# parklab/emsar

Hardware: AMD Instinct MI355X
Metric: EM iterations/s (higher is better)
Workload: dtype f64

## Files before the change

### emsar_amd/csrc/emsar_hip.hip

```cpp
#include <hip/hip_runtime.h>

#include <algorithm>
#include <chrono>
#include <cmath>
#include <cstdio>
#include <cstdlib>
#include <cstring>
#include <new>
#include <numeric>
#include <string>
#include <vector>

#include "../../include/emsar_hip.h"
#include "layout.hpp"
#include "layout_tiled.hpp"
#include "sets.hpp"
#include "boot_rng.hpp"
#include "internal.hpp"
#include "devmem.hpp"
#include "fit_index.hpp"

#include "kernels_common.hpp"
#include "kernels_csr.hpp"
#include "kernels_tiled.hpp"
#include "kernels_vector.hpp"
#include "kernels_sets.hpp"
#include "kernels_presence.hpp"
#include "kernels_cluster.hpp"
#include "kernels_boot.hpp"
#include "kernels_genes.hpp"
#include "kernels_quant.hpp"
#include "kernels_isoforms.hpp"
#include "kernels_fit.hpp"

using emsar::DevBuf;
using emsar::PinBuf;


// ... 17 lines not shown
};

struct GeneMap {
    bool have_genes = false;
    int32_t n_genes = 0;
    int64_t n_gene_chunks = 0, n_gene_multi = 0;
    DevBuf<int32_t> d_gene_blk;
    int32_t *d_gene_tx = nullptr, *d_chunk_beg = nullptr, *d_chunk_out = nullptr, *d_gene_multi = nullptr, *d_gene_of_lib = nullptr;
};

struct AdjEuma {
    DevBuf<int32_t> d_euma_t; int32_t nfl = 0; DevBuf<double> d_wf, d_adj;
};

struct RowWeights { DevBuf<int32_t> d_wgt, d_left_wgt; };

struct LayoutDev {
    DevBuf<void> d_row_ptr;
    DevBuf<int32_t> d_col;
    emsar::TiledLayout TL;
    DevBuf<Tile> d_tiles;
    DevBuf<Tile> d_utiles; int unit_stride = 1;
    DevBuf<uint32_t> d_units; int64_t n_units = 0;
    DevBuf<uint32_t> d_fwd, d_bwd;
    DevBuf<int32_t> d_far;
    DevBuf<uint64_t> d_left_ptr; DevBuf<int32_t> d_left_col; DevBuf<double> d_left_val;
    int64_t n_left = 0, n_tiles = 0, n_slots = 0;
    DevBuf<double> d_u;
    DevBuf<double> d_rowval;
};

struct TxVectors {
    DevBuf<double> d_den, d_acc;
    DevBuf<double> d_th[5];
    DevBuf<double> d_tmp[3];
    DevBuf<int32_t> d_itmp;
};

struct emsar_hip_ctx {
    int device = 0;
    int n_cu = 64;
    hipStream_t stream = nullptr;
    hipEvent_t ev0 = nullptr, ev1 = nullptr, ev2 = nullptr;
    hipStream_t side[3] = {nullptr, nullptr, nullptr};
    hipEvent_t ev_fork = nullptr, ev_join[3] = {nullptr, nullptr, nullptr};
    hipEvent_t ev_c0 = nullptr, ev_c1 = nullptr;
    std::string err;
    bool have_structure = false, have_sample = false;
    int layout = EMSAR_LAYOUT_CSR;
    int64_t n_rows = 0, nnz = 0;
    int32_t n_tx = 0;
    bool ptr64 = false;
    LayoutDev lay;
    TxVectors vec;
    GeneMap genes;
    AdjEuma euma;
    FitDev fit;
    bool weighted = false;
    RowWeights rw;
    SetsDev sets;
    double loglik_const = 0.0;
    DevBuf<Scal> d_scal;
    PinBuf<Scal> h_scal;
    int64_t bytes_formula = 0, bytes_stored = 0;
    int64_t tl_fwd_slots = 0, tl_n_fslices = 0;
    bool use_graph = true;
    bool det = false;
    double fx_mass = 0.0, fx_ll = 0.0;
    DevBuf<double> d_sqpart;
    int update_grid = 1024;
    int sq_grid = 256;
    int weighted_unit = 1;
    int tiled_multi = 1;
    std::vector<uint64_t> h_row_ptr;
    std::vector<int32_t> h_col, h_wgt;
    double sets_build_ms = 0.0;
};

namespace {

#define HIPCHK(call)                                                                                   \
    do {                                                                                               \
        hipError_t e_ = (call);                                                                        \
        if (e_ != hipSuccess) {                                                                        \
            ctx->err = std::string(#call) + ": " + hipGetErrorString(e_);                              \
            return e_ == hipErrorOutOfMemory ? EMSAR_HIP_ERR_OOM : EMSAR_HIP_ERR_HIP;                   \
        }                                                                                              \
    } while (0)

// ... 152 lines not shown
}



int choose_layout(int64_t n_rows, int &layout, bool &merge_rows) {
    merge_rows = (layout & EMSAR_LAYOUT_FLAG_MERGE_ROWS) != 0;
    layout &= ~EMSAR_LAYOUT_FLAG_MERGE_ROWS;
    if (layout != EMSAR_LAYOUT_AUTO && layout != EMSAR_LAYOUT_CSR && layout != EMSAR_LAYOUT_TILED) return EMSAR_HIP_ERR_ARG;
    if (layout == EMSAR_LAYOUT_AUTO) {
        layout = (n_rows < ((int64_t)1 << 32)) ? EMSAR_LAYOUT_TILED : EMSAR_LAYOUT_CSR;
        if (const char *e = getenv("EMSAR_HIP_LAYOUT")) { int v = atoi(e); if ((v == 1 || v == 3) && (v == 1 || n_rows < ((int64_t)1 << 32))) layout = v; }
    }
    return merge_rows && layout != EMSAR_LAYOUT_TILED ? EMSAR_HIP_ERR_ARG : EMSAR_HIP_OK;
}

struct UploadTrace {
    const bool on = getenv("EMSAR_HIP_DEBUG") != nullptr;
    const std::chrono::steady_clock::time_point t0 = std::chrono::steady_clock::now();
    void say(const char *what) const {
        if (on) fprintf(stderr, "upload_structure: %s after %.0f ms\n", what, std::chrono::duration<double, std::milli>(std::chrono::steady_clock::now() - t0).count());
    }
};

int upload_tiled(emsar_hip_ctx *ctx, const uint64_t *row_ptr, const int32_t *col_idx, bool merge_rows, const UploadTrace &trace) {
    auto &L = ctx->lay.TL;
    LayoutDev &D = ctx->lay;
    const size_t T = (size_t)ctx->n_tx;
    const int brc = emsar::build_tiled(ctx->n_rows, ctx->n_tx, row_ptr, col_idx, L, merge_rows);
    if (brc != 0) { ctx->err = "TILED layout builder: code " + std::to_string(brc); return EMSAR_HIP_ERR_ARG; }
    trace.say("layout built");
    D.n_tiles = (int64_t)L.tiles.size(); D.n_slots = L.n_slots(); D.n_left = (int64_t)L.left_row.size();
    HIPCHK(D.d_tiles.upload(L.tiles.data(), L.tiles.size()));
    HIPCHK(D.d_units.upload(L.unit_first.data(), L.unit_first.size()));
    D.n_units = L.unit_first.empty() ? 0 : (int64_t)L.unit_first.size() - 1;
    {
        emsar::UnitTables U;
        emsar::build_unit_tables(L, U);
        D.unit_stride = U.stride;
        HIPCHK(D.d_utiles.upload(U.utiles.data(), U.utiles.size()));
    }
    HIPCHK(D.d_fwd.upload(L.fwd.data(), L.fwd.size()));
    HIPCHK(D.d_bwd.upload(L.bwd.data(), L.bwd.size()));
    HIPCHK(D.d_far.upload(L.far_tid.data(), L.far_tid.size()));
    HIPCHK(D.d_left_ptr.upload(L.left_ptr.data(), L.left_ptr.size()));
    HIPCHK(D.d_left_col.upload(L.left_col.data(), L.left_col.size()));
    HIPCHK(D.d_u.alloc(T));
    HIPCHK(hipMemset(D.d_u, 0, T * 8));
    ctx->bytes_stored = (int64_t)L.fwd.size() * 4 + (int64_t)L.bwd.size() * 4 + (int64_t)L.far_tid.size() * 4 +
                        (int64_t)L.tiles.size() * 64 + (int64_t)L.left_col.size() * 4 + (int64_t)L.left_ptr.size() * 8;
    ctx->tl_fwd_slots = L.padded_slots; ctx->tl_n_fslices = L.n_fslices;
    emsar::u32_vec().swap(L.fwd); emsar::u32_vec().swap(L.bwd);
    std::vector<int32_t>().swap(L.left_col);
    HIPCHK(set_tiled_lds_attributes());
    { const char *pe = getenv("EMSAR_HIP_WEIGHTED_UNIT"); ctx->weighted_unit = pe ? atoi(pe) : 1; }
    { const char *pe = getenv("EMSAR_HIP_TILED_MULTI"); ctx->tiled_multi = pe ? atoi(pe) : 1; }
    { const char *pe = getenv("EMSAR_HIP_UPDATE_GRID"); if (pe && atoi(pe) >= 1) ctx->update_grid = atoi(pe); }
    { const char *pe = getenv("EMSAR_HIP_SQ_GRID"); if (pe && atoi(pe) >= 1) ctx->sq_grid = atoi(pe); }
    return EMSAR_HIP_OK;
}

int upload_csr(emsar_hip_ctx *ctx, const uint64_t *row_ptr, const int32_t *col_idx) {
    const int64_t n_rows = ctx->n_rows;
    if (ctx->ptr64) {
// ... 287 lines not shown
    HIPCHK(hipGetLastError());
    HIPCHK(hipMemcpyAsync(out, ctx->euma.d_adj, (size_t)ctx->n_rows * 8, hipMemcpyDeviceToHost, ctx->stream));
    HIPCHK(hipStreamSynchronize(ctx->stream));
    return EMSAR_HIP_OK;
}

int emsar_hip_get_info(const emsar_hip_ctx *ctx, emsar_hip_info *o) {
    if (!ctx || !o) return EMSAR_HIP_ERR_ARG;
    if (!ctx->have_structure) return EMSAR_HIP_ERR_STATE;
    memset(o, 0, sizeof(*o));
    o->n_rows = ctx->n_rows; o->nnz = ctx->nnz; o->n_tx = ctx->n_tx; o->device_id = ctx->device;
    o->layout = ctx->layout | ((ctx->layout == EMSAR_LAYOUT_TILED && ctx->lay.TL.merged) ? EMSAR_LAYOUT_FLAG_MERGE_ROWS : 0);
    if (ctx->layout == EMSAR_LAYOUT_TILED) {
        o->n_chunks = ctx->lay.n_tiles; o->n_slices = ctx->tl_n_fslices; o->padded_entries = ctx->tl_fwd_slots;
        o->far_entries = ctx->lay.TL.far_entries; o->window = emsar::kTileDict;
        o->tiled_entries = ctx->lay.TL.tiled_entries; o->tiled_ids = ctx->lay.TL.tiled_ids; o->renumbered = ctx->lay.TL.renum.applied ? 1 : 0;
        o->n_units = ctx->lay.n_units;
    }
    o->bytes_per_pass = ctx->bytes_formula;
    o->stored_bytes_per_pass = stored_bytes(ctx);
    return EMSAR_HIP_OK;
}

int emsar_hip_layout_selfcheck_tiled(int64_t n_rows, int32_t n_tx, const uint64_t *row_ptr, const int32_t *col_idx,
                                     int merge_rows, emsar_hip_info *info_out) {
    try {
        if (emsar::validate_csr(n_rows, n_tx, row_ptr, col_idx) != 0) return EMSAR_HIP_ERR_ARG;
        emsar::TiledLayout L;
        if (emsar::build_tiled(n_rows, n_tx, row_ptr, col_idx, L, merge_rows != 0) != 0) return EMSAR_HIP_ERR_ARG;
        int rc = emsar::check_tiled(L, row_ptr, col_idx);
        if (rc == 0) { emsar::UnitTables U; emsar::build_unit_tables(L, U); rc = emsar::check_unit_tables(L, U); }
        if (info_out) {
            memset(info_out, 0, sizeof(*info_out));
            info_out->n_rows = n_rows; info_out->nnz = L.nnz; info_out->n_tx = n_tx;
            info_out->layout = EMSAR_LAYOUT_TILED | (L.merged ? EMSAR_LAYOUT_FLAG_MERGE_ROWS : 0);
            info_out->n_chunks = (int64_t)L.tiles.size();
            info_out->n_slices = L.n_fslices;
            info_out->padded_entries = L.padded_slots; info_out->far_entries = L.far_entries; info_out->window = emsar::kTileDict;
            info_out->stored_bytes_per_pass = (int64_t)L.fwd.size() * 4 + (int64_t)L.bwd.size() * 4 +
                                              (int64_t)L.far_tid.size() * 4 + (int64_t)L.tiles.size() * 64 + (int64_t)L.left_col.size() * 4;
            info_out->bytes_per_pass = (int64_t)L.single_row.size();
            info_out->tiled_entries = L.tiled_entries; info_out->tiled_ids = L.tiled_ids; info_out->renumbered = L.renum.applied ? 1 : 0;
            info_out->n_units = L.unit_first.empty() ? 0 : (int64_t)L.unit_first.size() - 1;
        }
        return rc == 0 ? EMSAR_HIP_OK : EMSAR_HIP_ERR_ARG - 100 + rc;
    } catch (const std::bad_alloc &) { return EMSAR_HIP_ERR_OOM; }
// ... 32 lines not shown
```

### emsar_amd/csrc/kernels_tiled.hpp

```cpp
#pragma once

namespace {

#ifndef EMSAR_UE_BATCH
#define EMSAR_UE_BATCH 6
#endif
#ifndef EMSAR_UM_BATCH
#define EMSAR_UM_BATCH 6
#endif
constexpr int kTiledThreads = 256;
constexpr int kRPL = emsar::kRowsPerLane;
constexpr int kTiledWr = emsar::kTileSliceRows + 8;
constexpr int kTiledDictPad = emsar::kDictEntries;
constexpr int kBlk = emsar::kBlk;
constexpr int kTiledLdsDoubles = 2 * kTiledDictPad + emsar::kTileSlices * kTiledWr;

__device__ __forceinline__ double lds_at(const double *base, unsigned byte_off) {
    return *reinterpret_cast<const double *>(reinterpret_cast<const char *>(base) + byte_off);
}
__device__ __forceinline__ unsigned id_off(unsigned dword, int f) { return ((dword >> (10 * f)) & 0x3FFu) << 3; }

typedef int v4i_t __attribute__((ext_vector_type(4)));
__device__ __forceinline__ void load8_clamped(int4 (&q)[8], const int4 *e, int n) {
#pragma unroll
    for (int j = 0; j < 8; j++) {
        const v4i_t t = __builtin_nontemporal_load(reinterpret_cast<const v4i_t *>(e + (size_t)(j < n ? j : n - 1) * 64));
        q[j] = make_int4(t.x, t.y, t.z, t.w);
    }
}

template <int LO>
__device__ __forceinline__ void load4_clamped(int4 (&q)[8], const int4 *e, int n) {
#pragma unroll
    for (int j = LO; j < LO + 4; j++) {
        const v4i_t t = __builtin_nontemporal_load(reinterpret_cast<const v4i_t *>(e + (size_t)(j < n ? j : n - 1) * 64));
        q[j] = make_int4(t.x, t.y, t.z, t.w);
    }
}

typedef __attribute__((address_space(3))) const double lds_cdouble;
__device__ __forceinline__ unsigned lds_byte_addr(const void *p) { return (unsigned)(uintptr_t)p; }
template <int F>
__device__ __forceinline__ unsigned lds_id_addr(unsigned dword, unsigned base ) {
    unsigned a;
    asm("v_bfe_u32 %0, %1, %2, 10\n\tv_lshl_add_u32 %0, %0, 3, %3" : "=v"(a) : "v"(dword), "i"(10 * F), "s"(base));
    return a;
}
__device__ __forceinline__ double lds_ld(unsigned a) { return *reinterpret_cast<lds_cdouble *>(a); }
template <int H>
__device__ __forceinline__ void lds_addr6(const int4 t, unsigned base, unsigned (&a)[6]) {
    const unsigned d0 = (unsigned)(H ? t.z : t.x), d1 = (unsigned)(H ? t.w : t.y);
    a[0] = lds_id_addr<0>(d0, base); a[1] = lds_id_addr<1>(d0, base); a[2] = lds_id_addr<2>(d0, base);
    a[3] = lds_id_addr<0>(d1, base); a[4] = lds_id_addr<1>(d1, base); a[5] = lds_id_addr<2>(d1, base);
}

template <int BATCH = 12, int LO = 0, int HI = 8>
__device__ __forceinline__ void fwd_sum_regs(const int4 (&q)[8], int n, unsigned th_base, double (&S)[kRPL]) {
#pragma unroll
// ... 519 lines not shown
    BlockDict D;
    int4 A[8], B[8];
    block_dict_far_issue(far_tid + T.far_off, (int)T.far_n, D);
    block_dict_issue<MODE>(T, theta, D);
    if (W.has_slice) {
        load8_clamped(A, W.e, W.k < 8 ? W.k : 8);
        if (W.m > 0) load8_clamped(B, W.b, W.m < 8 ? W.m : 8);
    }
    if (V.lane < 8) V.w_s[emsar::kTileSliceRows + V.lane] = 0.0;
    LlAcc ll;
    tiled_stage<WEIGHTED, MODE, 0, N>(V, (int)blockIdx.x, T, W, A, B, D, ll);
    if (MODE == MODE_EM_LL) {
        double t = block_sum<kTiledThreads>(ll_value(ll), red);
        if (threadIdx.x == 0 && t != 0.0) ll_add(ll_out, t, fx.ll);
    }
}

template <bool WEIGHTED, int MODE, bool STAMP = false>
__global__ __launch_bounds__(kTiledThreads, 4) void k_pass_tiled_unit(const Tile *__restrict__ utiles, int stride, const int32_t *__restrict__ far_tid,
                                                                   const uint32_t *__restrict__ fwd, const uint32_t *__restrict__ bwd,
                                                                   
                                                                   const int32_t *__restrict__ wgt, const double *__restrict__ theta,
                                                                   double *__restrict__ acc, double *__restrict__ ll_out, Fx fx,
                                                                   unsigned long long *stamps = nullptr) {
    extern __shared__ __attribute__((aligned(16))) double lds[];
    __shared__ double red[kTiledThreads / 64];
    const int lane = threadIdx.x & 63;
    const int wave = __builtin_amdgcn_readfirstlane(threadIdx.x >> 6);
    double *th_w = lds, *acc_w = lds + kTiledDictPad, *w_s = lds + 2 * kTiledDictPad + wave * kTiledWr;
    unsigned long long ts0 = 0, ts1 = 0, ts2 = 0, te = 0, tm = 0, tr0 = 0;
    if (STAMP) { ts0 = stamp_now(); tr0 = stamp_real(); }
    const Tile *tiles = utiles + (size_t)blockIdx.x * (size_t)stride;
    BlockDict D;
    DTile T = tile_load(tiles);
    block_dict_far_issue(far_tid + T.far_off, (int)T.far_n, D);
    const int dict_near_n = (int)T.near_n, dict_lo = T.lo, dict_far_n = (int)T.far_n;
    const uint32_t dict_far_off = T.far_off;
    TileWave W = tile_wave(T, unit_slice(T, wave), lane, fwd, bwd);
    int4 A[8], B[8];
    load8_clamped(A, W.has_slice ? W.e : reinterpret_cast<const int4 *>(fwd), W.has_slice ? (W.k < 8 ? W.k : 8) : 1);
    block_dict_issue<MODE>(T, theta, D);
    if (lane < 8) w_s[emsar::kTileSliceRows + lane] = 0.0;
    block_dict_store(T, D, th_w, acc_w);
    vm_loads_landed();
    if (STAMP) ts1 = stamp_now();
    __syncthreads();
    if (STAMP) ts2 = stamp_now();
    LlAcc ll;
    int n_done = 0;
    for (int t = 0;; t++) {
        unsigned long long ta = 0, tb = 0;
        if (STAMP) ta = stamp_now();
        if (W.has_slice) {
            load8_clamped(B, W.b, W.m < 8 ? W.m : 8);
            tile_e_step<WEIGHTED, MODE>(W, A, (size_t)T.row_base + (size_t)W.slice * emsar::kTileSliceRows + lane, wgt, th_w, w_s, lane, ll);
// ... 54 lines not shown
```

### emsar_amd/csrc/layout_tiled.hpp

```cpp
#pragma once
#include <algorithm>
#include <thread>
#include <atomic>
#include <chrono>
#include <cstdio>
#include <cstddef>
#include <cstdint>
#include <cstdlib>
#include <cstring>
#include <functional>
#include <memory>
#include <new>
#include <system_error>
#include <utility>
#include <vector>

#include "layout.hpp"
#include "renumber.hpp"

namespace emsar {

constexpr int kTileSlices = 4;
constexpr int kRowsPerLane = 12;
constexpr int kTileSliceRows = 64 * kRowsPerLane;
// ... 859 lines not shown
struct UnitTables { std::vector<Tile> utiles; int stride = 1; };
inline void build_unit_tables(const TiledLayout &L, UnitTables &U) {
    const size_t nu = L.unit_first.empty() ? 0 : L.unit_first.size() - 1;
    int stride = 1;
    for (size_t u = 0; u < nu; u++) stride = std::max(stride, (int)(L.unit_first[u + 1] - L.unit_first[u]));
    U.stride = stride;
    Tile none;
    std::memset(&none, 0, sizeof none);
    U.utiles.assign(nu * (size_t)stride, none);
    for (size_t u = 0; u < nu; u++) {
        const uint32_t a = L.unit_first[u], b = L.unit_first[u + 1];
        for (uint32_t t = a; t < b; t++) U.utiles[u * (size_t)stride + (t - a)] = L.tiles[t];
    }
    if (getenv("EMSAR_HIP_DEBUG")) {
        std::vector<uint32_t> cnt((size_t)L.n_tx, 0);
        size_t slots = 0, with = 0; uint32_t mx = 0;
        for (size_t u = 0; u < nu; u++) {
            const Tile &T = L.tiles[L.unit_first[u]];
            for (uint32_t f = 0; f < T.far_n; f++) { cnt[(size_t)L.far_tid[(size_t)T.far_off + f]]++; slots++; }
        }
        for (uint32_t c : cnt) { with += c > 0; mx = std::max(mx, c); }
        fprintf(stderr, "unit tables: %zu units, stride %d, %zu far slots of %zu transcripts (most per transcript %u)\n", nu, stride, slots, with, mx);
    }
}

inline int check_unit_tables(const TiledLayout &L, const UnitTables &U) {
    const size_t nu = L.unit_first.empty() ? 0 : L.unit_first.size() - 1;
    if (U.stride < 1 || U.stride > kUnitMaxTiles) return -40;
    if (U.utiles.size() != nu * (size_t)U.stride) return -41;
    for (size_t u = 0; u < nu; u++) {
        const uint32_t a = L.unit_first[u], b = L.unit_first[u + 1];
        if (b - a > (uint32_t)U.stride) return -42;
        for (int j = 0; j < U.stride; j++) {
            const Tile &X = U.utiles[u * (size_t)U.stride + (size_t)j];
            if (a + (uint32_t)j < b) { if (std::memcmp(&X, &L.tiles[a + (uint32_t)j], sizeof(Tile)) != 0) return -43; }
            else if (X.n_slices != 0) return -44;
        }
    }
    return 0;
}

inline int check_tiled(const TiledLayout &L, const uint64_t *row_ptr, const int32_t *col_idx_in) {
    if (const int ext = check_tiled_extents(L)) return ext;
    std::vector<int32_t> mapped;
    const int32_t *col_idx = col_idx_in;
    if (!L.new_of_old.empty()) {
// ... 98 lines not shown
```

### emsar_amd/csrc/pass_launch.hpp

```cpp

namespace {

constexpr int64_t kPairMinTiles = 2048;
enum PassFamily { FAMILY_TILE, FAMILY_MULTI, FAMILY_UNIT };
struct PassKernel { PassFamily family; bool weighted; int mode; int n_multi;  };

PassKernel choose_pass_kernel(bool weighted, int mode, int64_t n_tiles, int tiled_multi, int weighted_unit) {
    if (mode == MODE_SCATTER) return {FAMILY_TILE, false, MODE_SCATTER, 0};
    const bool above = tiled_multi == 1 && n_tiles > kPairMinTiles;
    if (!weighted && (tiled_multi >= 2 || above)) {
        if (tiled_multi == 1 || tiled_multi == 5) return {FAMILY_UNIT, false, mode, 0};
        return {FAMILY_MULTI, false, mode, tiled_multi == 3 ? 3 : tiled_multi == 4 ? 4 : 2};
    }
    if (weighted && (weighted_unit == 2 || (weighted_unit == 1 && mode == MODE_EM)) && (tiled_multi == 5 || above)) {
        return {FAMILY_UNIT, true, mode, 0};
    }
    return {FAMILY_TILE, weighted, mode, 0};
}

template <bool B> using BoolC = std::integral_constant<bool, B>;
template <int M> using ModeC = std::integral_constant<int, M>;
template <class F> void with_em_mode(int mode, const F &f) { if (mode == MODE_EM_LL) f(ModeC<MODE_EM_LL>()); else f(ModeC<MODE_EM>()); }
template <class F> void with_em_variant(bool weighted, int mode, const F &f) {
    if (weighted) with_em_mode(mode, [&](auto md) { f(BoolC<true>(), md); });
    else with_em_mode(mode, [&](auto md) { f(BoolC<false>(), md); });
}

constexpr size_t kTiledLds = (size_t)kTiledLdsDoubles * sizeof(double);
struct PassArgs { const double *theta; double *acc, *ll_out; Fx fx; };

template <bool WT, int MD> void launch_tile(BoolC<WT>, ModeC<MD>, emsar_hip_ctx *ctx, const PassArgs &a) {
    const LayoutDev &L = ctx->lay;
    hipLaunchKernelGGL((k_pass_tiled<WT, MD>), dim3((unsigned)L.n_tiles), dim3(kTiledThreads), kTiledLds, ctx->stream, L.d_tiles, L.d_fwd, L.d_bwd,
                       L.d_far, ctx->rw.d_wgt, L.d_rowval, a.theta, a.acc, a.ll_out, a.fx);
}
template <bool WT, int MD, int N> void launch_multi(BoolC<WT>, ModeC<MD>, std::integral_constant<int, N>, emsar_hip_ctx *ctx, const PassArgs &a) {
    const LayoutDev &L = ctx->lay;
    hipLaunchKernelGGL((k_pass_tiled_multi<WT, MD, N>), dim3((unsigned)((L.n_tiles + N - 1) / N)), dim3(kTiledThreads), kTiledLds, ctx->stream, L.d_tiles,
                       (int)L.n_tiles, L.d_fwd, L.d_bwd, L.d_far, ctx->rw.d_wgt, a.theta, a.acc, a.ll_out, a.fx);
}
template <bool WT, int MD> void launch_unit(BoolC<WT>, ModeC<MD>, emsar_hip_ctx *ctx, const PassArgs &a) {
    const LayoutDev &L = ctx->lay;
    hipLaunchKernelGGL((k_pass_tiled_unit<WT, MD>), dim3((unsigned)L.n_units), dim3(kTiledThreads), kTiledLds, ctx->stream, L.d_utiles, L.unit_stride,
                       L.d_far, L.d_fwd, L.d_bwd, ctx->rw.d_wgt, a.theta, a.acc, a.ll_out, a.fx);
}
template <class PT, bool WT, int MD>
void launch_csr_rows(emsar_hip_ctx *ctx, unsigned max_grid, int64_t n_rows, const PT *row_ptr, const int32_t *col, const int32_t *wgt, const double *val, const PassArgs &a) {
    hipLaunchKernelGGL((k_pass_csr<PT, WT, MD>), dim3((unsigned)std::min<int64_t>((n_rows + 255) / 256, max_grid)), dim3(256), 0, ctx->stream, n_rows, row_ptr,
                       col, wgt, val, a.theta, a.acc, a.ll_out, a.fx);
}
template <bool WT, int MD> void launch_left(BoolC<WT>, ModeC<MD>, emsar_hip_ctx *ctx, const PassArgs &a) {
    const LayoutDev &L = ctx->lay;
    launch_csr_rows<uint64_t, WT, MD>(ctx, 8192, L.n_left, L.d_left_ptr, L.d_left_col, ctx->rw.d_left_wgt, L.d_left_val, a);
}
template <bool WT, int MD> void launch_csr(BoolC<WT>, ModeC<MD>, emsar_hip_ctx *ctx, const PassArgs &a) {
    const LayoutDev &L = ctx->lay;
    if (ctx->ptr64) launch_csr_rows<uint64_t, WT, MD>(ctx, 256 * 32, ctx->n_rows, (const uint64_t *)L.d_row_ptr.get(), L.d_col, ctx->rw.d_wgt, L.d_rowval, a);
    else launch_csr_rows<uint32_t, WT, MD>(ctx, 256 * 32, ctx->n_rows, (const uint32_t *)L.d_row_ptr.get(), L.d_col, ctx->rw.d_wgt, L.d_rowval, a);
}

hipError_t set_tiled_lds_attributes() {
    hipError_t e = hipSuccess;
    auto set = [&](auto *kernel) { if (e == hipSuccess) e = hipFuncSetAttribute((const void *)kernel, hipFuncAttributeMaxDynamicSharedMemorySize, (int)kTiledLds); };
    set(k_pass_tiled<false, MODE_SCATTER>);
    for (const bool weighted : {false, true})
        for (const int mode : {MODE_EM, MODE_EM_LL})
            with_em_variant(weighted, mode, [&](auto wt, auto md) { set(k_pass_tiled<wt(), md()>); set(k_pass_tiled_unit<wt(), md()>); });
// ... 54 lines not shown
        for (size_t w = 0; w < nw; w++) sum += (double)h[w * 8 + (size_t)i];
        out[i] = sum / (double)nw;
    }
    return EMSAR_HIP_OK;
}

}

extern "C" {

int emsar_hip_debug_tiled_stamps(emsar_hip_ctx *ctx, double *out) {
    if (!ctx || !out || ctx->layout != EMSAR_LAYOUT_TILED || !ctx->have_sample || ctx->weighted || ctx->lay.n_tiles == 0) return EMSAR_HIP_ERR_STATE;
    const LayoutDev &L = ctx->lay;
    const size_t nw = (size_t)L.n_tiles * (kTiledThreads / 64);
    std::vector<unsigned long long> h;
    const int rc = stamped_launch(ctx, (const void *)k_pass_tiled<false, MODE_EM, true>, nw, nw * 8, [&](unsigned long long *d) {
        hipLaunchKernelGGL((k_pass_tiled<false, MODE_EM, true>), dim3((unsigned)L.n_tiles), dim3(kTiledThreads), kTiledLds, ctx->stream, L.d_tiles, L.d_fwd, L.d_bwd,
                           L.d_far, ctx->rw.d_wgt, L.d_rowval, ctx->vec.d_th[0], ctx->vec.d_acc, &ctx->d_scal->ll[3].s[0].v, Fx{0.0, 0.0}, d);
    }, h, out);
    if (rc == EMSAR_HIP_OK) out[7] = (double)L.n_tiles;
    return rc;
}

int emsar_hip_debug_unit_stamps(emsar_hip_ctx *ctx, double *out, unsigned long long *timeline ) {
    if (!ctx || !out || ctx->layout != EMSAR_LAYOUT_TILED || !ctx->have_sample || ctx->weighted || ctx->lay.n_units == 0) return EMSAR_HIP_ERR_STATE;
    const LayoutDev &L = ctx->lay;
    const size_t nw = (size_t)L.n_units * (kTiledThreads / 64);
    std::vector<unsigned long long> h;
    const int rc = stamped_launch(ctx, (const void *)k_pass_tiled_unit<false, MODE_EM, true>, nw, nw * 8 + (size_t)L.n_units * 4, [&](unsigned long long *d) {
        hipLaunchKernelGGL((k_pass_tiled_unit<false, MODE_EM, true>), dim3((unsigned)L.n_units), dim3(kTiledThreads), kTiledLds, ctx->stream, L.d_utiles, L.unit_stride,
                           L.d_far, L.d_fwd, L.d_bwd, ctx->rw.d_wgt, ctx->vec.d_th[0], ctx->vec.d_acc, &ctx->d_scal->ll[3].s[0].v, Fx{0.0, 0.0}, d);
    }, h, out);
    if (rc != EMSAR_HIP_OK) return rc;
    if (timeline) std::copy(h.begin() + (std::ptrdiff_t)(nw * 8), h.end(), timeline);
    out[7] = (double)L.n_units;
    return EMSAR_HIP_OK;
}

int emsar_hip_debug_pass_kernel(int weighted, int mode, int64_t n_tiles, int tiled_multi, int weighted_unit, char *out, size_t cap) {
    if (!out || mode < MODE_EM || mode > MODE_SCATTER) return EMSAR_HIP_ERR_ARG;
    const PassKernel k = choose_pass_kernel(weighted != 0, mode, n_tiles, tiled_multi, weighted_unit);
    const char *const wt = k.weighted ? "true" : "false";
    const int len = k.family == FAMILY_MULTI  ? snprintf(out, cap, "k_pass_tiled_multi<%s, %d, %d>", wt, k.mode, k.n_multi)
                    : k.family == FAMILY_UNIT ? snprintf(out, cap, "k_pass_tiled_unit<%s, %d>", wt, k.mode)
                                              : snprintf(out, cap, "k_pass_tiled<%s, %d>", wt, k.mode);
    return len >= 0 && (size_t)len < cap ? EMSAR_HIP_OK : EMSAR_HIP_ERR_ARG;
}

}
```

### emsar_amd/hip.py

```python
import ctypes as C
import os

import numpy as np

_PKG = os.path.dirname(os.path.abspath(__file__))
_LIB_PATH = os.environ.get("EMSAR_HIP_LIB") or os.path.join(_PKG, "libemsar_hip.so")
_lib = None

LAYOUT_AUTO, LAYOUT_CSR, LAYOUT_TILED = 0, 1, 3
FLAG_MERGE_ROWS = 0x100

SYMBOLS = [
    "emsar_hip_create", "emsar_hip_destroy", "emsar_hip_strerror", "emsar_hip_last_error",
    "emsar_hip_upload_structure", "emsar_hip_upload_sample", "emsar_hip_solve",
    "emsar_hip_reset_theta", "emsar_hip_set_theta", "emsar_hip_get_theta", "emsar_hip_run_passes",
    "emsar_hip_ieuma", "emsar_hip_normalise", "emsar_hip_get_info",
    "emsar_hip_layout_selfcheck_tiled", "emsar_hip_sets_selfcheck", "emsar_hip_upload_euma", "emsar_hip_adj_euma", "emsar_hip_collapse_rows",
    "emsar_hip_set_deterministic", "emsar_hip_bootstrap", "emsar_hip_bootstrap_weights", "emsar_hip_bootstrap_draw_host",
    "emsar_hip_set_gene_map", "emsar_hip_gene_sums", "emsar_hip_bootstrap_genes",
    "emsar_hip_subsample", "emsar_hip_subsample_weights", "emsar_hip_subsample_draw_host",
    "emsar_hip_bootstrap_quantiles", "emsar_hip_quantiles_host",
    "emsar_hip_isoform_usage", "emsar_hip_isoform_usage_host", "emsar_hip_bootstrap_isoforms",
    "emsar_hip_model_fit", "emsar_hip_model_fit_host",
    "emsar_hip_presence", "emsar_hip_presence_pvalue_host",
]

PRESENCE_STATUS = ("TESTED", "ABSENT", "ESSENTIAL", "OUTSIDE", "NOT_RESIDENT", "UNCONVERGED")


class EmsarHipError(RuntimeError):
    def __init__(self, status, what, detail=""):
        self.status = status
        super().__init__("%s: %s (status %d)%s" % (what, _strerror(status), status, (" -- " + detail) if detail else ""))


class EmParams(C.Structure):
    _fields_ = [("max_iter", C.c_int32), ("accel", C.c_int32), ("tol", C.c_double), ("abs_floor", C.c_double),
                ("check_every", C.c_int32), ("set_mode", C.c_int32), ("count_floor", C.c_double), ("zero_cut", C.c_double), ("abs_step", C.c_double),
                ("newton_after", C.c_int32), ("reserved0", C.c_int32)]
# ... 96 lines not shown
    if _lib is not None:
        return _lib
    if not os.path.exists(_LIB_PATH):
        raise EmsarHipError(-4, "load_library", "%s missing: run python -m emsar_amd._build" % _LIB_PATH)
    L = C.CDLL(_LIB_PATH)
    vp, u64p, i32p, f64p = C.c_void_p, C.POINTER(C.c_uint64), C.POINTER(C.c_int32), C.POINTER(C.c_double)
    L.emsar_hip_create.argtypes = [C.POINTER(vp), C.c_int]
    L.emsar_hip_destroy.argtypes = [vp]
    L.emsar_hip_destroy.restype = None
    L.emsar_hip_strerror.argtypes = [C.c_int]
    L.emsar_hip_strerror.restype = C.c_char_p
    L.emsar_hip_last_error.argtypes = [vp]
    L.emsar_hip_last_error.restype = C.c_char_p
    L.emsar_hip_upload_structure.argtypes = [vp, C.c_int64, C.c_int32, u64p, i32p, C.c_int]
    L.emsar_hip_upload_sample.argtypes = [vp, i32p, f64p, f64p]
    L.emsar_hip_solve.argtypes = [vp, C.POINTER(EmParams), f64p, C.POINTER(EmStats)]
    L.emsar_hip_reset_theta.argtypes = [vp]
    L.emsar_hip_set_theta.argtypes = [vp, f64p]
    L.emsar_hip_get_theta.argtypes = [vp, f64p]
    L.emsar_hip_run_passes.argtypes = [vp, C.c_int32, C.POINTER(C.c_float), f64p]
    L.emsar_hip_ieuma.argtypes = [vp, f64p, f64p]
    L.emsar_hip_normalise.argtypes = [vp, f64p, f64p, C.c_int64, f64p, f64p, i32p]
    L.emsar_hip_get_info.argtypes = [vp, C.POINTER(Info)]
    L.emsar_hip_layout_selfcheck_tiled.argtypes = [C.c_int64, C.c_int32, u64p, i32p, C.c_int, C.POINTER(Info)]
    L.emsar_hip_set_deterministic.argtypes = [vp, C.c_int]
    L.emsar_hip_set_deterministic.restype = C.c_int
    L.emsar_hip_collapse_rows.argtypes = [vp, C.c_int64, C.c_int32, u64p, i32p, i32p, C.POINTER(C.c_int64), u64p, i32p, i32p, i32p,
                                          C.POINTER(CollapseStats)]
    L.emsar_hip_upload_euma.argtypes = [vp, i32p, C.c_int32]
    L.emsar_hip_adj_euma.argtypes = [vp, f64p, f64p]
    L.emsar_hip_sets_selfcheck.argtypes = [C.c_int64, C.c_int32, u64p, i32p, i32p, C.POINTER(SetsInfo)]
    L.emsar_hip_bootstrap.argtypes = [vp, C.POINTER(EmParams), C.c_uint64, C.c_int32, C.c_int32, f64p, f64p, f64p, f64p, C.POINTER(BootStats)]
    L.emsar_hip_bootstrap_weights.argtypes = [vp, C.c_uint64, C.c_int32, i32p]
    L.emsar_hip_bootstrap_draw_host.argtypes = [C.c_uint64, C.c_int32, C.c_int64, i32p, i32p]
    L.emsar_hip_set_gene_map.argtypes = [vp, C.c_int32, i32p]
    L.emsar_hip_gene_sums.argtypes = [vp, C.c_int32, f64p, f64p]
    L.emsar_hip_bootstrap_genes.argtypes = [vp, C.POINTER(EmParams), C.c_uint64, C.c_int32, C.c_int32, f64p, f64p, f64p, f64p,
                                            f64p, f64p, f64p, C.POINTER(BootStats)]
    L.emsar_hip_subsample.argtypes = [vp, C.POINTER(EmParams), C.c_uint64, C.c_int32, f64p, C.c_int32, f64p, f64p, f64p, f64p, f64p, f64p,
                                      f64p, f64p, f64p, C.POINTER(SubsampleStats)]
    L.emsar_hip_subsample_weights.argtypes = [vp, C.c_uint64, C.c_int32, C.c_double, i32p]
    L.emsar_hip_subsample_draw_host.argtypes = [C.c_uint64, C.c_int32, C.c_double, C.c_int64, i32p, i32p]
    L.emsar_hip_bootstrap_quantiles.argtypes = [vp, C.POINTER(EmParams), C.c_uint64, C.c_int32, C.c_int32, C.c_int32, f64p] + [f64p] * 12 + [
        C.POINTER(BootStats), C.POINTER(QuantileStats)]
    L.emsar_hip_quantiles_host.argtypes = [C.c_int32, C.c_int64, f64p, C.c_int32, f64p, f64p]
    L.emsar_hip_isoform_usage.argtypes = [vp, C.c_int32, f64p, f64p, i32p]
# ... 442 lines not shown
        ms = C.c_float(0)
        ll = C.c_double(0)
        self._chk(self._L.emsar_hip_run_passes(self._h, n, C.byref(ms), C.byref(ll) if want_loglik else None),
                  "run_passes")
        return (ms.value, ll.value) if want_loglik else ms.value

    def ieuma(self, row_L):
        row_L = _arr(row_L, np.float64)
        out = np.zeros(self.n_tx)
        self._chk(self._L.emsar_hip_ieuma(self._h, _p(row_L, C.c_double), _p(out, C.c_double)), "ieuma")
        return out

    def normalise(self, mean_fpkm, ieuma, total_read_count):
        m, ie = _arr(mean_fpkm, np.float64), _arr(ieuma, np.float64)
        tpm, ir = np.zeros(self.n_tx), np.zeros(self.n_tx)
        iri = np.zeros(self.n_tx, dtype=np.int32)
        self._chk(self._L.emsar_hip_normalise(self._h, _p(m, C.c_double), _p(ie, C.c_double), int(total_read_count),
                                              _p(tpm, C.c_double), _p(ir, C.c_double), _p(iri, C.c_int32)), "normalise")
        return tpm, ir, iri

    def info(self):
        i = Info()
        self._chk(self._L.emsar_hip_get_info(self._h, C.byref(i)), "get_info")
        return i.as_dict()
```

### include/emsar_hip.h

```cpp
#ifndef EMSAR_HIP_H
#define EMSAR_HIP_H

#include <stdint.h>

#ifdef __cplusplus
extern "C" {
#endif

typedef struct emsar_hip_ctx emsar_hip_ctx;

typedef enum {
    EMSAR_HIP_OK = 0,
    EMSAR_HIP_ERR_ARG = -1,
    EMSAR_HIP_ERR_NO_DEVICE = -2,
    EMSAR_HIP_ERR_OOM = -3,
    EMSAR_HIP_ERR_HIP = -4,
    EMSAR_HIP_ERR_STATE = -5,
    EMSAR_HIP_ERR_NUMERIC = -6
} emsar_hip_status;

typedef enum {
    EMSAR_LAYOUT_AUTO = 0,
    EMSAR_LAYOUT_CSR = 1,
    EMSAR_LAYOUT_TILED = 3
// ... 185 lines not shown
int emsar_hip_presence(emsar_hip_ctx *ctx, const emsar_em_params *p, int32_t n_query, const int32_t *query_tids ,
                       const emsar_presence_outputs *out , emsar_presence_stats *stats );
int emsar_hip_presence_pvalue_host(int64_t n, const double *lambda, double *p_out);

typedef struct {
    int64_t n_rows, nnz;
    int32_t n_tx;
    int32_t layout;
    int64_t n_chunks;
    int64_t n_slices;
    int64_t padded_entries;
    int64_t far_entries;
    int32_t window;
    int32_t device_id;
    int64_t bytes_per_pass;
    int64_t stored_bytes_per_pass;
    int64_t tiled_entries;
    int64_t tiled_ids;
    int64_t n_units;
    int32_t renumbered;
    int32_t reserved0;
} emsar_hip_info;
int emsar_hip_get_info(const emsar_hip_ctx *ctx, emsar_hip_info *out);

int emsar_hip_layout_selfcheck_tiled(int64_t n_rows, int32_t n_tx, const uint64_t *row_ptr, const int32_t *col_idx,
                                     int merge_rows, emsar_hip_info *info_out);

typedef struct {
    int64_t n_components;
    int64_t sets_resident[3];
    int64_t max_lds_bytes[3];
    int64_t sets_streamed;
    int64_t tids_closed, tids_resident, tids_streamed;
    int64_t rows_in, rows_stored;
    int64_t sets_cluster, tids_cluster, max_lds_cluster;
} emsar_hip_sets_info;
int emsar_hip_sets_selfcheck(int64_t n_rows, int32_t n_tx, const uint64_t *row_ptr, const int32_t *col_idx,
                             const int32_t *row_weight, emsar_hip_sets_info *info_out);

#ifdef __cplusplus
}
#endif
#endif
```

Baseline: 9616.

## Alternate tiled unit sweep order across passes to reuse cached index data

Result: no change. 9687 (median of 6 runs) (+0.7%).

```diff
diff --git a/emsar_amd/csrc/emsar_hip.hip b/emsar_amd/csrc/emsar_hip.hip
--- a/emsar_amd/csrc/emsar_hip.hip
+++ b/emsar_amd/csrc/emsar_hip.hip
@@ -14,6 +14,7 @@
 #include "../../include/emsar_hip.h"
 #include "layout.hpp"
 #include "layout_tiled.hpp"
+#include "sweep_order.hpp"
 #include "sets.hpp"
 #include "boot_rng.hpp"
 #include "internal.hpp"
@@ -77,6 +78,8 @@
     DevBuf<Tile> d_tiles;
     DevBuf<Tile> d_utiles; int unit_stride = 1;
     DevBuf<uint32_t> d_units; int64_t n_units = 0;
+    DevBuf<uint32_t> d_order[2];
+    int64_t sweep_head_units = 0, sweep_group_units = 0, sweep_reuse_bytes = 0;
     DevBuf<uint32_t> d_fwd, d_bwd;
     DevBuf<int32_t> d_far;
     DevBuf<uint64_t> d_left_ptr; DevBuf<int32_t> d_left_col; DevBuf<double> d_left_val;
@@ -120,6 +123,7 @@
     int64_t bytes_formula = 0, bytes_stored = 0;
     int64_t tl_fwd_slots = 0, tl_n_fslices = 0;
     bool use_graph = true;
+    int sweep_phase = 0;
     bool det = false;
     double fx_mass = 0.0, fx_ll = 0.0;
     DevBuf<double> d_sqpart;
@@ -318,6 +322,39 @@
     }
 };
 
+emsar::SweepKnobs read_sweep_knobs() {
+    auto knob = [](const char *name, int64_t dflt) { const char *e = getenv(name); const long long v = e ? atoll(e) : -1; return e && v >= 0 ? (int64_t)v : dflt; };
+    emsar::SweepKnobs K;
+    K.reuse_bytes = 1024 * knob("EMSAR_HIP_SWEEP_REUSE_KB", emsar::kSweepReuseKB);
+    K.head_bytes = 1024 * knob("EMSAR_HIP_SWEEP_HEAD_KB", emsar::kSweepHeadKB);
+    K.min_units = knob("EMSAR_HIP_SWEEP_MIN_UNITS", emsar::kSweepMinUnits);
+    return K;
+}
+int upload_sweep_order(emsar_hip_ctx *ctx, const emsar::SweepKnobs &K, bool same_phase = false) {
+    LayoutDev &D = ctx->lay;
+    ctx->sweep_phase = 0;
+    D.d_order[0] = DevBuf<uint32_t>(); D.d_order[1] = DevBuf<uint32_t>();
+    D.sweep_head_units = D.sweep_group_units = D.sweep_reuse_bytes = 0;
+    std::vector<int64_t> work, bytes;
+    emsar::unit_profile(D.TL, work, bytes);
+    emsar::SweepOrder S;
+    const bool on = emsar::build_sweep_order(work, bytes, K, S);
+    if (getenv("EMSAR_HIP_DEBUG")) {
+        fprintf(stderr, "sweep order: %zu units, slot-model span of the layout's order %.1f us", work.size(), emsar::sweep_slot_span(work, nullptr));
+        if (on) fprintf(stderr, "; head %zu units (%.1f MB), groups %zu + %zu units (%.1f + %.1f MB), reuse distance %.1f MB, span of the two phases %.1f / %.1f us\n",
+                        S.n_head, (double)S.head_bytes / 1e6, S.n_group[0], S.n_group[1], (double)S.group_bytes[0] / 1e6, (double)S.group_bytes[1] / 1e6,
+                        (double)S.reuse_distance() / 1e6, emsar::sweep_slot_span(work, S.phase[0].data()), emsar::sweep_slot_span(work, S.phase[1].data()));
+        else fprintf(stderr, "; no rotation\n");
+    }
+    if (!on) return EMSAR_HIP_OK;
+    for (int p = 0; p < 2; p++) {
+        if (S.phase[p].size() != (size_t)D.n_units) { ctx->err = "sweep order: a table of the wrong length"; return EMSAR_HIP_ERR_STATE; }
+        HIPCHK(D.d_order[p].upload(S.phase[same_phase ? 0 : p].data(), S.phase[p].size()));
+    }
+    D.sweep_head_units = (int64_t)S.n_head; D.sweep_group_units = (int64_t)std::min(S.n_group[0], S.n_group[1]); D.sweep_reuse_bytes = S.reuse_distance();
+    return EMSAR_HIP_OK;
+}
+
 int upload_tiled(emsar_hip_ctx *ctx, const uint64_t *row_ptr, const int32_t *col_idx, bool merge_rows, const UploadTrace &trace) {
     auto &L = ctx->lay.TL;
     LayoutDev &D = ctx->lay;
@@ -335,6 +372,7 @@
         D.unit_stride = U.stride;
         HIPCHK(D.d_utiles.upload(U.utiles.data(), U.utiles.size()));
     }
+    if (const int rc = upload_sweep_order(ctx, read_sweep_knobs())) return rc;
     HIPCHK(D.d_fwd.upload(L.fwd.data(), L.fwd.size()));
     HIPCHK(D.d_bwd.upload(L.bwd.data(), L.bwd.size()));
     HIPCHK(D.d_far.upload(L.far_tid.data(), L.far_tid.size()));
@@ -668,6 +706,37 @@
     return EMSAR_HIP_OK;
 }
 
+int emsar_hip_get_sweep_info(const emsar_hip_ctx *ctx, int64_t *out) {
+    if (!ctx || !out) return EMSAR_HIP_ERR_ARG;
+    if (!ctx->have_structure) return EMSAR_HIP_ERR_STATE;
+    out[0] = ctx->lay.sweep_head_units; out[1] = ctx->lay.sweep_group_units; out[2] = ctx->lay.sweep_reuse_bytes;
+    return EMSAR_HIP_OK;
+}
+
+int emsar_hip_debug_set_sweep(emsar_hip_ctx *ctx, int64_t reuse_kb, int64_t head_kb, int64_t min_units, int same_phase) {
+    if (!ctx || reuse_kb < 0 || head_kb < 0 || min_units < 0) return EMSAR_HIP_ERR_ARG;
+    if (!ctx->have_structure || ctx->layout != EMSAR_LAYOUT_TILED) return EMSAR_HIP_ERR_STATE;
+    HIPCHK(hipSetDevice(ctx->device));
+    HIPCHK(hipStreamSynchronize(ctx->stream));
+    emsar::SweepKnobs K;
+    K.reuse_bytes = 1024 * reuse_kb; K.head_bytes = 1024 * head_kb; K.min_units = min_units;
+    try { return upload_sweep_order(ctx, K, same_phase != 0); } catch (const std::bad_alloc &) { return EMSAR_HIP_ERR_OOM; }
+}
+
+int emsar_hip_debug_unit_profile(int64_t n_rows, int32_t n_tx, const uint64_t *row_ptr, const int32_t *col_idx, int merge_rows,
+                                 int64_t cap, int64_t *work, int64_t *bytes, int64_t *n_units) {
+    try {
+        if (!n_units || emsar::validate_csr(n_rows, n_tx, row_ptr, col_idx) != 0) return EMSAR_HIP_ERR_ARG;
+        emsar::TiledLayout L;
+        if (emsar::build_tiled(n_rows, n_tx, row_ptr, col_idx, L, merge_rows != 0) != 0) return EMSAR_HIP_ERR_ARG;
+        std::vector<int64_t> w, b;
+        emsar::unit_profile(L, w, b);
+        *n_units = (int64_t)w.size();
+        if (work && bytes && cap >= (int64_t)w.size()) { std::copy(w.begin(), w.end(), work); std::copy(b.begin(), b.end(), bytes); }
+        return EMSAR_HIP_OK;
+    } catch (const std::bad_alloc &) { return EMSAR_HIP_ERR_OOM; }
+}
+
 int emsar_hip_layout_selfcheck_tiled(int64_t n_rows, int32_t n_tx, const uint64_t *row_ptr, const int32_t *col_idx,
                                      int merge_rows, emsar_hip_info *info_out) {
     try {
diff --git a/emsar_amd/csrc/kernels_tiled.hpp b/emsar_amd/csrc/kernels_tiled.hpp
--- a/emsar_amd/csrc/kernels_tiled.hpp
+++ b/emsar_amd/csrc/kernels_tiled.hpp
@@ -21,10 +21,17 @@
 __device__ __forceinline__ unsigned id_off(unsigned dword, int f) { return ((dword >> (10 * f)) & 0x3FFu) << 3; }
 
 typedef int v4i_t __attribute__((ext_vector_type(4)));
+__device__ __forceinline__ v4i_t index_load(const v4i_t *p) {
+#ifdef EMSAR_HIP_TEMPORAL_INDEX
+    return *p;
+#else
+    return __builtin_nontemporal_load(p);
+#endif
+}
 __device__ __forceinline__ void load8_clamped(int4 (&q)[8], const int4 *e, int n) {
 #pragma unroll
     for (int j = 0; j < 8; j++) {
-        const v4i_t t = __builtin_nontemporal_load(reinterpret_cast<const v4i_t *>(e + (size_t)(j < n ? j : n - 1) * 64));
+        const v4i_t t = index_load(reinterpret_cast<const v4i_t *>(e + (size_t)(j < n ? j : n - 1) * 64));
         q[j] = make_int4(t.x, t.y, t.z, t.w);
     }
 }
@@ -33,7 +40,7 @@
 __device__ __forceinline__ void load4_clamped(int4 (&q)[8], const int4 *e, int n) {
 #pragma unroll
     for (int j = LO; j < LO + 4; j++) {
-        const v4i_t t = __builtin_nontemporal_load(reinterpret_cast<const v4i_t *>(e + (size_t)(j < n ? j : n - 1) * 64));
+        const v4i_t t = index_load(reinterpret_cast<const v4i_t *>(e + (size_t)(j < n ? j : n - 1) * 64));
         q[j] = make_int4(t.x, t.y, t.z, t.w);
     }
 }
@@ -599,6 +606,7 @@
                                                                    
                                                                    const int32_t *__restrict__ wgt, const double *__restrict__ theta,
                                                                    double *__restrict__ acc, double *__restrict__ ll_out, Fx fx,
+                                                                   const uint32_t *__restrict__ order ,
                                                                    unsigned long long *stamps = nullptr) {
     extern __shared__ __attribute__((aligned(16))) double lds[];
     __shared__ double red[kTiledThreads / 64];
@@ -607,7 +615,8 @@
     double *th_w = lds, *acc_w = lds + kTiledDictPad, *w_s = lds + 2 * kTiledDictPad + wave * kTiledWr;
     unsigned long long ts0 = 0, ts1 = 0, ts2 = 0, te = 0, tm = 0, tr0 = 0;
     if (STAMP) { ts0 = stamp_now(); tr0 = stamp_real(); }
-    const Tile *tiles = utiles + (size_t)blockIdx.x * (size_t)stride;
+    const unsigned unit = order ? order[blockIdx.x] : blockIdx.x;
+    const Tile *tiles = utiles + (size_t)unit * (size_t)stride;
     BlockDict D;
     DTile T = tile_load(tiles);
     block_dict_far_issue(far_tid + T.far_off, (int)T.far_n, D);
diff --git a/emsar_amd/csrc/layout_tiled.hpp b/emsar_amd/csrc/layout_tiled.hpp
--- a/emsar_amd/csrc/layout_tiled.hpp
+++ b/emsar_amd/csrc/layout_tiled.hpp
@@ -905,6 +905,17 @@
         for (uint32_t c : cnt) { with += c > 0; mx = std::max(mx, c); }
         fprintf(stderr, "unit tables: %zu units, stride %d, %zu far slots of %zu transcripts (most per transcript %u)\n", nu, stride, slots, with, mx);
     }
+}
+
+inline void unit_profile(const TiledLayout &L, std::vector<int64_t> &work, std::vector<int64_t> &bytes) {
+    const size_t nu = L.unit_first.empty() ? 0 : L.unit_first.size() - 1;
+    work.assign(nu, 0); bytes.assign(nu, 0);
+    for (size_t u = 0; u < nu; u++)
+        for (uint32_t t = L.unit_first[u]; t < L.unit_first[u + 1]; t++) {
+            const Tile &T = L.tiles[t];
+            work[u] += tile_work(T);
+            for (int s = 0; s < (int)T.n_slices; s++) bytes[u] += 1024 * ((int64_t)T.k[s] + (int64_t)T.m[s]);
+        }
 }
 
 inline int check_unit_tables(const TiledLayout &L, const UnitTables &U) {
diff --git a/emsar_amd/csrc/pass_launch.hpp b/emsar_amd/csrc/pass_launch.hpp
--- a/emsar_amd/csrc/pass_launch.hpp
+++ b/emsar_amd/csrc/pass_launch.hpp
@@ -41,8 +41,10 @@
 }
 template <bool WT, int MD> void launch_unit(BoolC<WT>, ModeC<MD>, emsar_hip_ctx *ctx, const PassArgs &a) {
     const LayoutDev &L = ctx->lay;
+    const uint32_t *order = L.d_order[ctx->sweep_phase].get();
+    ctx->sweep_phase ^= 1;
     hipLaunchKernelGGL((k_pass_tiled_unit<WT, MD>), dim3((unsigned)L.n_units), dim3(kTiledThreads), kTiledLds, ctx->stream, L.d_utiles, L.unit_stride,
-                       L.d_far, L.d_fwd, L.d_bwd, ctx->rw.d_wgt, a.theta, a.acc, a.ll_out, a.fx);
+                       L.d_far, L.d_fwd, L.d_bwd, ctx->rw.d_wgt, a.theta, a.acc, a.ll_out, a.fx, order);
 }
 template <class PT, bool WT, int MD>
 void launch_csr_rows(emsar_hip_ctx *ctx, unsigned max_grid, int64_t n_rows, const PT *row_ptr, const int32_t *col, const int32_t *wgt, const double *val, const PassArgs &a) {
@@ -143,19 +145,23 @@
     return rc;
 }
 
-int emsar_hip_debug_unit_stamps(emsar_hip_ctx *ctx, double *out, unsigned long long *timeline ) {
+int emsar_hip_debug_unit_stamps_phase(emsar_hip_ctx *ctx, int phase, double *out, unsigned long long *timeline ) {
+    if (phase < 0 || phase > 1) return EMSAR_HIP_ERR_ARG;
     if (!ctx || !out || ctx->layout != EMSAR_LAYOUT_TILED || !ctx->have_sample || ctx->weighted || ctx->lay.n_units == 0) return EMSAR_HIP_ERR_STATE;
     const LayoutDev &L = ctx->lay;
     const size_t nw = (size_t)L.n_units * (kTiledThreads / 64);
     std::vector<unsigned long long> h;
     const int rc = stamped_launch(ctx, (const void *)k_pass_tiled_unit<false, MODE_EM, true>, nw, nw * 8 + (size_t)L.n_units * 4, [&](unsigned long long *d) {
         hipLaunchKernelGGL((k_pass_tiled_unit<false, MODE_EM, true>), dim3((unsigned)L.n_units), dim3(kTiledThreads), kTiledLds, ctx->stream, L.d_utiles, L.unit_stride,
-                           L.d_far, L.d_fwd, L.d_bwd, ctx->rw.d_wgt, ctx->vec.d_th[0], ctx->vec.d_acc, &ctx->d_scal->ll[3].s[0].v, Fx{0.0, 0.0}, d);
+                           L.d_far, L.d_fwd, L.d_bwd, ctx->rw.d_wgt, ctx->vec.d_th[0], ctx->vec.d_acc, &ctx->d_scal->ll[3].s[0].v, Fx{0.0, 0.0}, L.d_order[phase].get(), d);
     }, h, out);
     if (rc != EMSAR_HIP_OK) return rc;
     if (timeline) std::copy(h.begin() + (std::ptrdiff_t)(nw * 8), h.end(), timeline);
     out[7] = (double)L.n_units;
     return EMSAR_HIP_OK;
+}
+int emsar_hip_debug_unit_stamps(emsar_hip_ctx *ctx, double *out, unsigned long long *timeline) {
+    return emsar_hip_debug_unit_stamps_phase(ctx, ctx ? ctx->sweep_phase : 0, out, timeline);
 }
 
 int emsar_hip_debug_pass_kernel(int weighted, int mode, int64_t n_tiles, int tiled_multi, int weighted_unit, char *out, size_t cap) {
diff --git a/emsar_amd/csrc/sweep_order.hpp b/emsar_amd/csrc/sweep_order.hpp
--- /dev/null
+++ b/emsar_amd/csrc/sweep_order.hpp
@@ -0,0 +1,75 @@
+#pragma once
+#include <algorithm>
+#include <cstddef>
+#include <cstdint>
+#include <functional>
+#include <queue>
+#include <vector>
+
+namespace emsar {
+
+constexpr int64_t kSweepReuseKB = 64000, kSweepHeadKB = 40000, kSweepMinUnits = 1024;
+
+struct SweepKnobs {
+    int64_t reuse_bytes = 0;
+    int64_t head_bytes = 0;
+    int64_t min_units = kSweepMinUnits;
+};
+
+struct SweepOrder {
+    std::vector<uint32_t> phase[2];
+    size_t n_head = 0, n_group[2] = {0, 0};
+    int64_t head_bytes = 0, group_bytes[2] = {0, 0};
+    bool on() const { return !phase[0].empty(); }
+    int64_t reuse_distance() const { return head_bytes + std::max(group_bytes[0], group_bytes[1]); }
+};
+
+inline bool build_sweep_order(const std::vector<int64_t> &work, const std::vector<int64_t> &bytes, const SweepKnobs &K, SweepOrder &out) {
+    out = SweepOrder();
+    const size_t n = work.size();
+    if (bytes.size() != n || K.reuse_bytes <= 0 || (int64_t)n <= K.min_units || n < 2) return false;
+    int64_t total = 0;
+    for (const int64_t b : bytes) total += b;
+    if (total <= K.reuse_bytes) return false;
+    size_t nh = 0;
+    int64_t hb = 0;
+    while (nh < n && hb + bytes[nh] <= K.head_bytes) hb += bytes[nh++];
+    const int64_t budget = K.reuse_bytes - hb;
+    if (budget <= 0) return false;
+    size_t g = n;
+    int64_t gb = 0;
+    while (g > nh && gb + bytes[g - 1] <= 2 * budget) gb += bytes[--g];
+    std::vector<int64_t> alt(n + 2, 0);
+    for (size_t i = n; i-- > g;) alt[i] = bytes[i] + alt[i + 2];
+    while (g < n && (alt[g] > budget || alt[g + 1] > budget)) g++;
+    if (n - g < 2) return false;
+    std::vector<uint32_t> hand[2];
+    for (size_t i = g; i < n; i++) hand[(i - g) & 1].push_back((uint32_t)i);
+    for (int p = 0; p < 2; p++) {
+        std::vector<uint32_t> &o = out.phase[p];
+        o.reserve(n);
+        for (size_t i = 0; i < nh; i++) o.push_back((uint32_t)i);
+        o.insert(o.end(), hand[p].begin(), hand[p].end());
+        for (size_t i = nh; i < g; i++) o.push_back((uint32_t)i);
+        o.insert(o.end(), hand[1 - p].begin(), hand[1 - p].end());
+    }
+    out.n_head = nh; out.head_bytes = hb;
+    for (int p = 0; p < 2; p++) { out.n_group[p] = hand[p].size(); out.group_bytes[p] = alt[g + (size_t)p]; }
+    return true;
+}
+
+struct SlotModel { int slots = 1024; double fixed_us = 9.8, per_work_us = 1.834e-4, gap_us = 1.7; };
+inline double sweep_slot_span(const std::vector<int64_t> &work, const uint32_t *order, const SlotModel &M = SlotModel()) {
+    std::priority_queue<double, std::vector<double>, std::greater<double>> free_at;
+    double span = 0.0;
+    for (size_t i = 0; i < work.size(); i++) {
+        double start = 0.0;
+        if ((int)free_at.size() >= M.slots) { start = free_at.top() + M.gap_us; free_at.pop(); }
+        const double end = start + M.fixed_us + M.per_work_us * (double)work[order ? order[i] : i];
+        free_at.push(end);
+        span = std::max(span, end);
+    }
+    return span;
+}
+
+}
diff --git a/emsar_amd/hip.py b/emsar_amd/hip.py
--- a/emsar_amd/hip.py
+++ b/emsar_amd/hip.py
@@ -14,7 +14,7 @@
     "emsar_hip_create", "emsar_hip_destroy", "emsar_hip_strerror", "emsar_hip_last_error",
     "emsar_hip_upload_structure", "emsar_hip_upload_sample", "emsar_hip_solve",
     "emsar_hip_reset_theta", "emsar_hip_set_theta", "emsar_hip_get_theta", "emsar_hip_run_passes",
-    "emsar_hip_ieuma", "emsar_hip_normalise", "emsar_hip_get_info",
+    "emsar_hip_ieuma", "emsar_hip_normalise", "emsar_hip_get_info", "emsar_hip_get_sweep_info",
     "emsar_hip_layout_selfcheck_tiled", "emsar_hip_sets_selfcheck", "emsar_hip_upload_euma", "emsar_hip_adj_euma", "emsar_hip_collapse_rows",
     "emsar_hip_set_deterministic", "emsar_hip_bootstrap", "emsar_hip_bootstrap_weights", "emsar_hip_bootstrap_draw_host",
     "emsar_hip_set_gene_map", "emsar_hip_gene_sums", "emsar_hip_bootstrap_genes",
@@ -157,6 +157,8 @@
     L.emsar_hip_ieuma.argtypes = [vp, f64p, f64p]
     L.emsar_hip_normalise.argtypes = [vp, f64p, f64p, C.c_int64, f64p, f64p, i32p]
     L.emsar_hip_get_info.argtypes = [vp, C.POINTER(Info)]
+    if hasattr(L, "emsar_hip_get_sweep_info"):
+        L.emsar_hip_get_sweep_info.argtypes = [vp, C.POINTER(C.c_int64)]
     L.emsar_hip_layout_selfcheck_tiled.argtypes = [C.c_int64, C.c_int32, u64p, i32p, C.c_int, C.POINTER(Info)]
     L.emsar_hip_set_deterministic.argtypes = [vp, C.c_int]
     L.emsar_hip_set_deterministic.restype = C.c_int
@@ -645,4 +647,9 @@
     def info(self):
         i = Info()
         self._chk(self._L.emsar_hip_get_info(self._h, C.byref(i)), "get_info")
-        return i.as_dict()
+        d = i.as_dict()
+        sweep = (C.c_int64 * 3)()
+        if hasattr(self._L, "emsar_hip_get_sweep_info"):
+            self._chk(self._L.emsar_hip_get_sweep_info(self._h, sweep), "get_sweep_info")
+        d["sweep_head_units"], d["sweep_group_units"], d["sweep_reuse_bytes"] = (int(x) for x in sweep)
+        return d
diff --git a/include/emsar_hip.h b/include/emsar_hip.h
--- a/include/emsar_hip.h
+++ b/include/emsar_hip.h
@@ -231,6 +231,7 @@
     int32_t reserved0;
 } emsar_hip_info;
 int emsar_hip_get_info(const emsar_hip_ctx *ctx, emsar_hip_info *out);
+int emsar_hip_get_sweep_info(const emsar_hip_ctx *ctx, int64_t out[3]);
 
 int emsar_hip_layout_selfcheck_tiled(int64_t n_rows, int32_t n_tx, const uint64_t *row_ptr, const int32_t *col_idx,
                                      int merge_rows, emsar_hip_info *info_out);
```
